# vLAR-group/DM-NeRF

Hardware: AMD Instinct MI355X
Metric: rays/sec (render) at 640x480, 64+128 samples (higher is better)
Workload: dtype f32; 1 GPU; DM-SR 'study' 640x480 synthetic camera, dm_nerf render, 64 coarse + 128 fine samples, 4096-ray chunk per step per GPU, det sampling, ins_num=13, random-init weights; chunks_per_band=75, ragged_chunk_rays=0, parallelism=ray-sharded x1

## Files before the change

dm_nerf_amd/csrc/mlp_common.h:

```cpp
#pragma once
#include <hip/hip_runtime.h>

#include <type_traits>
#include <utility>

#include "layout.h"

namespace dmn {

typedef float f32x16 __attribute__((ext_vector_type(16)));
typedef float f32x4 __attribute__((ext_vector_type(4)));

__device__ __forceinline__ f32x16 mfma32(float a, float b, f32x16 c) {
    return __builtin_amdgcn_mfma_f32_32x32x2f32(a, b, c, 0, 0, 0);
}

typedef __amdgpu_buffer_rsrc_t rsrc_t;
typedef unsigned int u32x4 __attribute__((ext_vector_type(4)));

__device__ __forceinline__ float relu1(float x) {
    const int xi = (int)__float_as_uint(x);
    return __uint_as_float((unsigned)(xi > 0 ? xi : 0));
}
__device__ __forceinline__ f32x16 relu16(f32x16 v) {
    f32x16 r;
#pragma unroll
    for (int i = 0; i < 16; ++i) r[i] = relu1(v[i]);
    return r;
}

__device__ __forceinline__ double rev_of(float v) { return (double)v * 0.15915494309189535; }

__device__ __forceinline__ double sin_rev_d(double t, int k, int quarter) {
    double g = t * (double)(1 << k) + 0.25 * (double)quarter;
    g = g - __builtin_rint(g);
    const double ag = __builtin_fabs(g);
    const double gf = ag > 0.25 ? 0.5 - ag : ag;
    const double x = gf * 6.283185307179586;
    const double x2 = x * x;
    double p = 1.0 / 1307674368000.0;
    p = __builtin_fma(p, x2, -1.0 / 6227020800.0);
    p = __builtin_fma(p, x2, 1.0 / 39916800.0);
    p = __builtin_fma(p, x2, -1.0 / 362880.0);
    p = __builtin_fma(p, x2, 1.0 / 5040.0);
    p = __builtin_fma(p, x2, -1.0 / 120.0);
    p = __builtin_fma(p, x2, 1.0 / 6.0);
    const double s = x - x * x2 * p;
    return __builtin_copysign(s, g);
}
__device__ __forceinline__ float sin_rev(double t, int k, int quarter) { return (float)sin_rev_d(t, k, quarter); }

template <int L, int NV>
__device__ __forceinline__ void encode(const float (&v)[3], f32x16 (&out)[NV], int half) {
    static_assert(NV * 16 >= 2 + 3 * L, "encoding registers too small");
#pragma unroll
    for (int i = 0; i < NV; ++i) out[i] = (f32x16)(0.f);
    out[0][0] = half ? v[1] : v[0];
    out[0][1] = half ? 0.f : v[2];
#pragma unroll
    for (int c = 0; c < 3; ++c) {
        const double t = rev_of(v[c]);
        double sn = sin_rev_d(t, 0, 0), cs = sin_rev_d(t, 0, 1);
#pragma unroll
        for (int k = 0; k < L; ++k) {
            const int p = 2 + 3 * k + c;
            out[p >> 4][p & 15] = (float)(half ? cs : sn);
            const double s_old = sn, t2 = s_old + s_old;
            sn = t2 * cs;
            cs = __builtin_fma(-t2, s_old, 1.0);
        }
    }
}

template <int L, int NV>
__device__ __forceinline__ void load_encoded(const float* __restrict__ e, f32x16 (&out)[NV], int half) {
#pragma unroll
    for (int i = 0; i < NV; ++i) out[i] = (f32x16)(0.f);
    out[0][0] = e[half];
    out[0][1] = half ? 0.f : e[2];
#pragma unroll
    for (int k = 0; k < L; ++k) {
#pragma unroll
        for (int c = 0; c < 3; ++c) {
            const int p = 2 + 3 * k + c;
            out[p >> 4][p & 15] = e[3 + 6 * k + 3 * half + c];
        }
    }
}


#ifndef DMN_STORE_AUX
#define DMN_STORE_AUX 0
#endif
#ifdef DMN_NO_ACT_STORES
#define DMN_ACT_STORE_B32(...) ((void)0)
#else
#define DMN_ACT_STORE_B32(...) __builtin_amdgcn_raw_buffer_store_b32(__VA_ARGS__)
#endif
struct RowIO {
    rsrc_t rs;
    unsigned soff;
};

__device__ __forceinline__ unsigned f2u(float x) { return __float_as_uint(x); }

__device__ __forceinline__ rsrc_t uniform_rsrc(const float* base, int64_t n_floats) {
    const unsigned long long p = reinterpret_cast<unsigned long long>(base);
    const unsigned lo = __builtin_amdgcn_readfirstlane((unsigned)p);
    const unsigned hi = __builtin_amdgcn_readfirstlane((unsigned)(p >> 32));
    const unsigned nb = __builtin_amdgcn_readfirstlane((unsigned)(n_floats * 4));
    float* q = reinterpret_cast<float*>(((unsigned long long)hi << 32) | lo);
    return __builtin_amdgcn_make_buffer_rsrc(q, 0, (int)nb, 0x00020000);
}

__device__ __forceinline__ RowIO make_rowio(const float* base, int R, int64_t Mp, int64_t blk, int lane, int ob0 = 0) {
    RowIO io;
    const unsigned long long p = reinterpret_cast<unsigned long long>(base);
    const unsigned lo = __builtin_amdgcn_readfirstlane((unsigned)p);
    const unsigned hi = __builtin_amdgcn_readfirstlane((unsigned)(p >> 32));
    float* q = reinterpret_cast<float*>(((unsigned long long)hi << 32) | lo);
    io.rs = __builtin_amdgcn_make_buffer_rsrc(q, 4, 64, 1 << 23);
    (void)Mp;
#ifdef DMN_ACT_STORE_HOT
    blk &= 7;
#endif
    io.soff = __builtin_amdgcn_readfirstlane((unsigned)(blk * R * 128 + ob0 * 4096));
    (void)lane;
    return io;
}

__device__ __forceinline__ constexpr int run_off(int b, int r) { return (32 * b + 8 * (r >> 2) + 2 * (r & 3)) * 128; }

template <int NB>
__device__ __forceinline__ void store_rows(const RowIO& io, const f32x16 (&v)[NB]) {
#pragma unroll
    for (int b = 0; b < NB; ++b) {
#pragma unroll
        for (int r = 0; r < 16; ++r)
            DMN_ACT_STORE_B32(f2u(v[b][r]), io.rs, run_off(0, r), (int)(io.soff + b * 4096), DMN_STORE_AUX);
    }
}

template <int L, int NV>
__device__ __forceinline__ void store_encoded_rows(const float* base, int64_t Mp, int64_t blk, int lane,
                                                   const f32x16 (&e)[NV]) {
    constexpr int R = 3 + 6 * L;
    const int half = lane >> 5, j = lane & 31;
    rsrc_t rs = uniform_rsrc(base, (int64_t)R * Mp);
    const int v0 = (int)((blk * R * 32 + j) * 4);
    __builtin_amdgcn_raw_buffer_store_b32(f2u(e[0][0]), rs, v0 + half * 128, 0, 0);
    if (half == 0) __builtin_amdgcn_raw_buffer_store_b32(f2u(e[0][1]), rs, v0 + 2 * 128, 0, 0);
    const int v3 = v0 + 3 * half * 128;
#pragma unroll
    for (int k = 0; k < L; ++k) {
#pragma unroll
        for (int c = 0; c < 3; ++c) {
            const int p = 2 + 3 * k + c;
            __builtin_amdgcn_raw_buffer_store_b32(f2u(e[p >> 4][p & 15]), rs, v3 + ((3 + 6 * k + c) * 128) % 4096, ((3 + 6 * k + c) * 128) / 4096 * 4096, 0);
        }
    }
}


constexpr int SLOT_FLOATS = QUARTER_FLOATS;
constexpr int RING_FLOATS = 2 * SLOT_FLOATS;
constexpr int LDS_FLOATS = RING_FLOATS + TAB_FLOATS;
constexpr int DMA_PER_QUARTER = 16;

#define DMN_GAS __attribute__((address_space(1)))
#define DMN_LAS __attribute__((address_space(3)))

struct WStream {
    rsrc_t rs;
    unsigned voff;
    float* ring;
    int wave;
    unsigned off;
    int cslot;
    f32x4 pre[8];
};

__device__ __forceinline__ void ws_init(WStream& ws, const float* blob, int64_t blob_floats, float* ring, int lane, int wave,
                                        int64_t stream_float_off) {
    ws.rs = uniform_rsrc(blob, blob_floats);
    ws.wave = __builtin_amdgcn_readfirstlane(wave);
    ws.voff = (unsigned)(lane * 16 + ws.wave * 1024);
    ws.ring = ring;
    ws.off = __builtin_amdgcn_readfirstlane((unsigned)(stream_float_off * 4));
    ws.cslot = 0;
}

__device__ __forceinline__ void ws_fetch_piece(const WStream& ws, int i) {
    float* dst = ws.ring + (ws.cslot ^ 1) * SLOT_FLOATS + ws.wave * 256 + i * 1024;
    __builtin_amdgcn_raw_ptr_buffer_load_lds(ws.rs, (DMN_LAS void*)dst, 16, (int)ws.voff, (int)(ws.off + i * 4096), 0, 0);
}
__device__ __forceinline__ void ws_fetch(WStream& ws) {
#pragma unroll
    for (int i = 0; i < DMA_PER_QUARTER; ++i) ws_fetch_piece(ws, i);
    ws.off += QUARTER_FLOATS * 4;
}

__device__ __forceinline__ void ws_fetch_first(WStream& ws) {
    ws.cslot = 1;
    ws_fetch(ws);
    ws.cslot = 0;
}

__device__ __forceinline__ unsigned lds_addr(const void* p) {
    return (unsigned)(unsigned long long)(DMN_LAS const void*)p;
}
#ifndef DMN_TILE_RC
#define DMN_TILE_RC "v"
#endif
#ifndef DMN_CARRY_RC
#define DMN_CARRY_RC DMN_TILE_RC
#endif
template <int OFF, bool CARRY = false>
__device__ __forceinline__ void lds_read16_async(f32x4& v, unsigned addr) {
    static_assert(OFF >= 0 && OFF < 65536 && OFF % 16 == 0, "ds_read_b128 offset field");
    if constexpr (CARRY) asm volatile("ds_read_b128 %0, %1 offset:%2" : "=" DMN_CARRY_RC(v) : "v"(addr), "n"(OFF));
    else asm volatile("ds_read_b128 %0, %1 offset:%2" : "=" DMN_TILE_RC(v) : "v"(addr), "n"(OFF));
}
template <class F, int... I>
__device__ __forceinline__ void static_for_impl(F&& f, std::integer_sequence<int, I...>) {
    (f(std::integral_constant<int, I>{}), ...);
}
template <int N, class F>
__device__ __forceinline__ void static_for(F&& f) {
    static_for_impl(f, std::make_integer_sequence<int, N>{});
}
template <int N, bool CARRY = false, int NV>
__device__ __forceinline__ void lds_wait(f32x4 (&v)[NV]) {
    __builtin_amdgcn_s_waitcnt(0xC07F | (N << 8));
#pragma unroll
    for (int i = 0; i < NV; ++i) {
        if constexpr (CARRY) asm volatile("" : "+" DMN_CARRY_RC(v[i]));
        else asm volatile("" : "+" DMN_TILE_RC(v[i]));
    }
}

template <int NYOUNGER = 0>
__device__ __forceinline__ void ws_handover() {
    __builtin_amdgcn_s_waitcnt(0x0F70 | (NYOUNGER & 15) | ((NYOUNGER >> 4) << 14));
    asm volatile("" ::: "memory");
    __builtin_amdgcn_s_barrier();
    asm volatile("" ::: "memory");
}

struct NoSide {
    __device__ __forceinline__ void operator()(int) const {}
};

template <int OB>
__device__ __forceinline__ void ws_prime(WStream& ws, int lane) {
    asm volatile("s_waitcnt vmcnt(0) lgkmcnt(0)" ::: "memory");
    __builtin_amdgcn_s_barrier();
    asm volatile("" ::: "memory");
    const unsigned s0 = lds_addr(ws.ring + ws.cslot * SLOT_FLOATS) + lane * 16;
    static_for<OB>([&](auto ic) {
        constexpr int ob = decltype(ic)::value;
        lds_read16_async<ob * 1024, true>(ws.pre[ob], s0);
    });
    lds_wait<0, true>(ws.pre);
}

template <int G0, int NG, int OB, int NEXT_OB, bool ZERO = false, int NSIDE = 0, int NB, class Side = NoSide>
__device__ __forceinline__ void gemm_quarter(WStream& ws, const f32x16 (&B)[NB], f32x16 (&acc)[OB], int lane, Side&& side = Side()) {
    static_assert(NB * 16 >= (G0 + NG) * 4, "B operand too small");
    static_assert(NG * OB <= 64, "more than one quarter");
    constexpr int GM = 4 * OB;
    constexpr int Q = NG * GM;
    constexpr int P = (Q / 4) / DMA_PER_QUARTER > 0 ? (Q / 4) / DMA_PER_QUARTER : 1;
    static_assert(OB + (DMA_PER_QUARTER - 1) * P < Q - GM, "DMA pieces must be issued before the last group");
    static_assert(NG >= 2 && NEXT_OB <= GM && NEXT_OB <= 8, "hand-over does not fit the last group");
    constexpr int S0 = OB + DMA_PER_QUARTER * P;
    constexpr int SP = NSIDE > 0 ? ((Q - GM - S0) / NSIDE >= 3 ? 3 : ((Q - GM - S0) / NSIDE >= 1 ? (Q - GM - S0) / NSIDE : 1)) : 1;
    static_assert(NSIDE == 0 || (S0 + (NSIDE - 1) * SP < Q - GM && NSIDE <= 63), "side operations do not fit before the last group");
    const unsigned s0 = lds_addr(ws.ring + ws.cslot * SLOT_FLOATS) + lane * 16;
    const unsigned s1 = lds_addr(ws.ring + (ws.cslot ^ 1) * SLOT_FLOATS) + lane * 16;
    f32x4 a[2][OB];
#pragma unroll
    for (int ob = 0; ob < OB; ++ob) a[0][ob] = ws.pre[ob];
    static_for<NG>([&](auto gc) {
        constexpr int gl = decltype(gc)::value;
        lds_wait<0>(a[gl & 1]);
        if constexpr (gl == NG - 1 && NEXT_OB > 0) ws_handover<NSIDE>();
        __builtin_amdgcn_sched_barrier(0);
        static_for<GM>([&](auto ic) {
            constexpr int i = decltype(ic)::value;
            constexpr int kk = i / OB, ob = i % OB, M = gl * GM + i;
            constexpr int p = (G0 + gl) * 4 + kk;
            if constexpr (gl + 1 < NG && i < OB)
                lds_read16_async<((gl + 1) * OB + i) * 1024>(a[(gl + 1) & 1][i], s0);
            if constexpr (gl == NG - 1 && i < NEXT_OB) lds_read16_async<i * 1024, true>(ws.pre[i], s1);
            if constexpr (M >= OB && (M - OB) % P == 0 && (M - OB) / P < DMA_PER_QUARTER) ws_fetch_piece(ws, (M - OB) / P);
            if constexpr (NSIDE > 0 && M >= S0 && (M - S0) % SP == 0 && (M - S0) / SP < NSIDE) side((M - S0) / SP);
            if constexpr (ZERO && G0 + gl == 0 && kk == 0) acc[ob] = mfma32(a[gl & 1][ob][kk], B[p >> 4][p & 15], (f32x16)(0.f));
            else acc[ob] = mfma32(a[gl & 1][ob][kk], B[p >> 4][p & 15], acc[ob]);
            __builtin_amdgcn_sched_barrier(0);
        });
    });
    if constexpr (NEXT_OB > 0) __builtin_amdgcn_s_waitcnt(0xC07F);
    ws.off += QUARTER_FLOATS * 4;
    ws.cslot ^= 1;
}

template <int OB>
__device__ __forceinline__ void init_bias_lds(const float* tab_seg, f32x16 (&acc)[OB], int half) {
#pragma unroll
    for (int ob = 0; ob < OB; ++ob) {
        const f32x4* b4 = reinterpret_cast<const f32x4*>(tab_seg + (ob * 2 + half) * 16);
#pragma unroll
        for (int q = 0; q < 4; ++q) {
            const f32x4 v = b4[q];
            acc[ob][4 * q + 0] = v[0]; acc[ob][4 * q + 1] = v[1];
            acc[ob][4 * q + 2] = v[2]; acc[ob][4 * q + 3] = v[3];
        }
    }
}

template <int NB>
__device__ __forceinline__ void pack_mask(const f32x16 (&h)[NB], unsigned (&m)[NB / 2]) {
#pragma unroll
    for (int w = 0; w < NB / 2; ++w) m[w] = 0;
#pragma unroll
    for (int i = 0; i < 32; ++i) {
#pragma unroll
        for (int w = 0; w < NB / 2; ++w) {
            const int p = 32 * w + i;
            const float x = h[p >> 4][p & 15];
            asm volatile("v_cmp_lt_f32 vcc, 0, %1\n\tv_addc_co_u32 %0, vcc, %0, %0, vcc" : "+v"(m[w]) : "v"(x) : "vcc");
        }
    }
}

template <int NB>
__device__ __forceinline__ void apply_mask(f32x16 (&d)[NB], const unsigned (&m)[NB / 2], const f32x16 (&g)[NB]) {
#pragma unroll
    for (int p = 0; p < NB * 16; ++p) {
        const unsigned keep = (unsigned)__builtin_amdgcn_sbfe((int)m[p >> 5], 31 - (p & 31), 1);
        d[p >> 4][p & 15] = __uint_as_float(__float_as_uint(g[p >> 4][p & 15]) & keep);
    }
}

template <int NB>
__device__ __forceinline__ void store_row_one(const RowIO& io, const f32x16 (&v)[NB], int p) {
    DMN_ACT_STORE_B32(f2u(v[p >> 4][p & 15]), io.rs, run_off(0, p & 15), (int)(io.soff + (p >> 4) * 4096), DMN_STORE_AUX);
}

template <int P0, int NP, int NB>
__device__ __forceinline__ void store_rows_part(const RowIO& io, const f32x16 (&v)[NB]) {
#pragma unroll
    for (int p = P0; p < P0 + NP; ++p)
        DMN_ACT_STORE_B32(f2u(v[p >> 4][p & 15]), io.rs, run_off(0, p & 15), (int)(io.soff + (p >> 4) * 4096), DMN_STORE_AUX);
}

}
```

dm_nerf_amd/csrc/mlp_fwd_density.hip:

```cpp
#include <hip/hip_runtime.h>

#include "../../include/dmnerf_hip.h"
#include "common.h"
#include "layout.h"
#include "mlp_common.h"

using namespace dmn;

namespace {

constexpr int DENSITY_QUARTERS = 1 + 5 * 4 + 1 + 2 * 4 + 1;
static_assert(DENSITY_QUARTERS <= N_QUARTERS - 2 * 4, "the look-ahead quarter must exist in the fused-heads blob as well");

struct DensityArgs {
    const float* blob;
    BlobLayout L;
    const float* rays_o;
    const float* rays_d;
    const float* z;
    float* sigma;
    int64_t M;
    int S;
};

__global__ __launch_bounds__(256) void mlp_fwd_density_kernel(const DensityArgs a) {
    extern __shared__ __attribute__((aligned(16))) float lds[];
    float* const tab = lds + RING_FLOATS;
    const int lane = threadIdx.x & 63;
    const int half = lane >> 5;
    const int wave = __builtin_amdgcn_readfirstlane(threadIdx.x >> 6);
    const int64_t nblk = (a.M + 31) / 32;
    const int64_t blk_raw = (int64_t)blockIdx.x * 4 + wave;
    const int64_t blk = blk_raw < nblk ? blk_raw : nblk - 1;
    auto fresh = [](int x) -> int { asm volatile("" : "+v"(x)); return x; };
    const int64_t m_in = blk * 32 + (lane & 31);
    const int64_t m = m_in < a.M ? m_in : a.M - 1;

    const float* __restrict__ blob = a.blob;
    const BlobLayout& L = a.L;

    float pt[3];
    {
        const int64_t n = m / a.S;
        const float ox = a.rays_o[n * 3 + 0], oy = a.rays_o[n * 3 + 1], oz = a.rays_o[n * 3 + 2];
        const float dx = a.rays_d[n * 3 + 0], dy = a.rays_d[n * 3 + 1], dz = a.rays_d[n * 3 + 2];
        const float zv = a.z[m];
        pt[0] = ox + dx * zv; pt[1] = oy + dy * zv; pt[2] = oz + dz * zv;
    }
    f32x16 pe[2];
    f32x4 tabv[TAB_FLOATS / 1024];
    {
        const f32x4* src = reinterpret_cast<const f32x4*>(blob) + threadIdx.x;
#pragma unroll
        for (int k = 0; k < TAB_FLOATS / 1024; ++k) tabv[k] = src[k * 256];
    }
    WStream ws;
    ws_init(ws, blob, L.stream + (int64_t)DENSITY_QUARTERS * QUARTER_FLOATS, lds, lane, wave, L.stream);
    ws_fetch_first(ws);
    encode<POS_L, 2>(pt, pe, half);
    {
        f32x4* dst = reinterpret_cast<f32x4*>(tab) + threadIdx.x;
#pragma unroll
        for (int k = 0; k < TAB_FLOATS / 1024; ++k) dst[k * 256] = tabv[k];
    }

    f32x16 h[8], acc[8];
    ws_prime<8>(ws, lane);
    init_bias_lds<8>(tab + L.b0, acc, half);
    gemm_quarter<0, 8, 8, 8>(ws, pe, acc, lane);
#pragma unroll
    for (int b = 0; b < 8; ++b) h[b] = relu16(acc[b]);

#pragma nounroll
    for (int st = 0; st < 7; ++st) {
        init_bias_lds<8>(tab + L.b_stage + st * (int)bias_floats(8), acc, half);
        gemm_quarter<0, 8, 8, 8>(ws, h, acc, lane);
        gemm_quarter<8, 8, 8, 8>(ws, h, acc, lane);
        gemm_quarter<16, 8, 8, 8>(ws, h, acc, lane);
        gemm_quarter<24, 8, 8, 8>(ws, h, acc, lane);
        if (st == 4) {
            gemm_quarter<0, 8, 8, 8>(ws, pe, acc, lane);
        }
#pragma unroll
        for (int b = 0; b < 8; ++b) h[b] = relu16(acc[b]);
    }
    const f32x4* wd = reinterpret_cast<const f32x4*>(tab + L.w_den + fresh(half) * 128);
    float part = 0.f;
#pragma unroll
    for (int i = 0; i < 32; ++i) {
        const f32x4 w = wd[i];
#pragma unroll
        for (int j = 0; j < 4; ++j) {
            const int p = 4 * i + j;
            part = fmaf(h[p >> 4][p & 15], w[j], part);
        }
    }
    const float sigma = part + __shfl_xor(part, 32) + tab[L.b_den];
    const int64_t ms = blk * 32 + (fresh(lane) & 31);
    if (ms < a.M && fresh(half) == 0) a.sigma[ms] = sigma;
}

}

extern "C" int dmnerf_mlp_fwd_rays_density(const float* d_blob, int ins_num, const float* d_rays_o,
                                           const float* d_rays_d, const float* d_z, int64_t N, int S,
                                           float* d_sigma, void* stream) {
    if (ins_num < 1 || ins_num + 1 > DMNERF_MAX_LOGITS) return dmn_fail(DMNERF_E_ARG, "mlp_fwd_rays_density: ins_num %d unsupported", ins_num);
    if (N < 0 || S < 1) return dmn_fail(DMNERF_E_ARG, "mlp_fwd_rays_density: bad N=%lld S=%d", (long long)N, S);
    if (N == 0) return DMNERF_OK;
    if (!d_blob || !d_rays_o || !d_rays_d || !d_z || !d_sigma) return dmn_fail(DMNERF_E_ARG, "mlp_fwd_rays_density: null pointer");
    DensityArgs a{};
    a.blob = d_blob; a.L = make_layout(ins_num); a.rays_o = d_rays_o; a.rays_d = d_rays_d; a.z = d_z;
    a.sigma = d_sigma; a.M = N * S; a.S = S;
    const int64_t nblk = (a.M + 31) / 32;
    const int64_t grid = (nblk + 3) / 4;
    if (grid > 0x7fffffffLL) return dmn_fail(DMNERF_E_ARG, "mlp_fwd_rays_density: %lld samples is too many for one launch", (long long)a.M);
    constexpr size_t lds_bytes = (size_t)LDS_FLOATS * sizeof(float);
    static DmnOncePerDevice once;
    if (hipError_t e = once.run([] { return hipFuncSetAttribute((const void*)mlp_fwd_density_kernel,
                                                                hipFuncAttributeMaxDynamicSharedMemorySize, (int)lds_bytes); }); e != hipSuccess)
        return dmn_fail_hip(e, "mlp_fwd_rays_density: hipFuncSetAttribute");
    hipLaunchKernelGGL(mlp_fwd_density_kernel, dim3((unsigned)grid), dim3(256), lds_bytes, (hipStream_t)stream, a);
    return dmn_check_launch("mlp_fwd_rays_density");
}
```

dm_nerf_amd/csrc/mlp_fwd_impl.h:

```cpp
#pragma once
#include <hip/hip_runtime.h>

#include "../../include/dmnerf_hip.h"
#include "common.h"
#include "layout.h"
#include "mlp_common.h"

#ifdef DMN_FWD_TRACE
extern long long* g_dmn_fwd_trace;
#endif

using namespace dmn;

namespace {

constexpr int PARK_FLOATS = 4096;

struct MlpArgs {
    const float* blob;
    BlobLayout L;
    const float* rays_o;
    const float* rays_d;
    const float* z;
    const float* x;
    float* raw;
    float* save;
    int64_t M;
    int S;
#ifdef DMN_FWD_TRACE
    long long* trace;
#endif
};
#ifdef DMN_FWD_TRACE
#define DMN_STAMP(k) do { if (a.trace && threadIdx.x == 0) { a.trace[8 * blockIdx.x + (k)] = (long long)clock64(); if ((k) == 0) a.trace[8 * blockIdx.x + 7] = (long long)wall_clock64(); } } while (0)
#else
#define DMN_STAMP(k) do {} while (0)
#endif

template <int OBI, bool EMBEDDED, bool SAVE, bool FUSED = false>
__global__ __launch_bounds__(256) void mlp_fwd_kernel(const MlpArgs a) {
    extern __shared__ __attribute__((aligned(16))) float lds[];
    float* const tab = lds + RING_FLOATS;
    DMN_STAMP(0);
    const int lane = threadIdx.x & 63;
    const int half = lane >> 5;
    const int wave = __builtin_amdgcn_readfirstlane(threadIdx.x >> 6);
    const int64_t nblk = (a.M + 31) / 32;
    const int64_t blk_raw = (int64_t)blockIdx.x * 4 + wave;
    const bool wave_active = blk_raw < nblk;
    const int64_t blk = wave_active ? blk_raw : nblk - 1;
    auto fresh = [](int x) -> int { asm volatile("" : "+v"(x)); return x; };
    auto sample_of_lane = [&]() -> int64_t { return blk * 32 + (fresh(lane) & 31); };
    const int64_t m_in = blk * 32 + (lane & 31);
    const int64_t m = m_in < a.M ? m_in : a.M - 1;
    auto park = [&]() -> f32x4* { return reinterpret_cast<f32x4*>(lds + LDS_FLOATS + wave * (PARK_FLOATS / 4)) + lane; };

    const float* __restrict__ blob = a.blob;
    const BlobLayout& L = a.L;

    float pt[3], vd[3];
    const float* xr = nullptr;
    if constexpr (EMBEDDED) {
        xr = a.x + m * (POS_CH + DIR_CH);
    } else {
        const int64_t n = m / a.S;
        const float ox = a.rays_o[n * 3 + 0], oy = a.rays_o[n * 3 + 1], oz = a.rays_o[n * 3 + 2];
        const float dx = a.rays_d[n * 3 + 0], dy = a.rays_d[n * 3 + 1], dz = a.rays_d[n * 3 + 2];
        const float zv = a.z[m];
        pt[0] = ox + dx * zv; pt[1] = oy + dy * zv; pt[2] = oz + dz * zv;
        const float nrm = sqrtf(dx * dx + dy * dy + dz * dz);
        vd[0] = dx / nrm; vd[1] = dy / nrm; vd[2] = dz / nrm;
    }
    f32x16 pe[2];
    f32x16 de[1];
    if constexpr (EMBEDDED) {
        load_encoded<POS_L, 2>(xr, pe, half);
        load_encoded<DIR_L, 1>(xr + POS_CH, de, half);
    }
    f32x4 tabv[TAB_FLOATS / 1024];
    {
        const f32x4* src = reinterpret_cast<const f32x4*>(blob) + threadIdx.x;
#pragma unroll
        for (int k = 0; k < TAB_FLOATS / 1024; ++k) tabv[k] = src[k * 256];
    }
    WStream ws;
    ws_init(ws, blob, L.total, lds, lane, wave, L.stream);
    ws_fetch_first(ws);
    if constexpr (!EMBEDDED) {
        encode<POS_L, 2>(pt, pe, half);
        encode<DIR_L, 1>(vd, de, half);
    }
    {
        f32x4* dst = reinterpret_cast<f32x4*>(tab) + threadIdx.x;
#pragma unroll
        for (int k = 0; k < TAB_FLOATS / 1024; ++k) dst[k * 256] = tabv[k];
    }

    const SaveLayout SL = make_save_layout(a.M);
    const int64_t MP = save_row_len(a.M);
    const int srows = 1;
    rsrc_t bits_rs;
    int bits_voff = 0;
    if constexpr (SAVE) {
        bits_rs = uniform_rsrc(a.save + SL.bits, (int64_t)srows * (BITS_WORDS_PER_BLOCK / 32) * MP);
        bits_voff = (int)((blk * BITS_WORDS_PER_BLOCK + lane * 4) * 4);
    }

    DMN_STAMP(1);
    f32x16 h[8], acc[8];
    auto save_mask8 = [&](int layer) {
        unsigned m[4];
        pack_mask<8>(h, m);
        u32x4 v = {m[0], m[1], m[2], m[3]};
        __builtin_amdgcn_raw_buffer_store_b128(v, bits_rs, bits_voff + layer * 1024, 0, 0);
    };
    ws_prime<8>(ws, lane);
    if constexpr (SAVE) {
        store_encoded_rows<POS_L, 2>(a.save + SL.pe, srows * MP, blk, lane, pe);
        store_encoded_rows<DIR_L, 1>(a.save + SL.de, srows * MP, blk, lane, de);
    }
#pragma unroll
    for (int q = 0; q < 4; ++q) {
        const f32x4 v = {de[0][4 * q + 0], de[0][4 * q + 1], de[0][4 * q + 2], de[0][4 * q + 3]};
        park()[q * 64] = v;
    }
    init_bias_lds<8>(tab + L.b0, acc, half);
    gemm_quarter<0, 8, 8, 8>(ws, pe, acc, lane);
#pragma unroll
    for (int b = 0; b < 8; ++b) h[b] = relu16(acc[b]);
    if constexpr (SAVE) save_mask8(0);

    DMN_STAMP(2);
    float sigma = 0.f, rgb_out[3] = {0.f, 0.f, 0.f};

    auto stage = [&](int st, auto next_ob, auto save_h) {
        constexpr int NEXT = decltype(next_ob)::value;
        constexpr bool SAVE_H = SAVE && decltype(save_h)::value;
        RowIO hio;
        if constexpr (SAVE) hio = make_rowio(a.save + SL.h + (int64_t)(st < 8 ? st : 7) * 256 * MP, 256, (st < 8 ? srows : 0) * MP, blk, lane);
        init_bias_lds<8>(tab + L.b_stage + st * (int)bias_floats(8), acc, half);
        constexpr int NS = SAVE_H ? 43 : 0;
        auto st_h = [&](int k0) { return [&, k0](int k) { store_row_one(hio, h, k0 + k); }; };
        gemm_quarter<0, 8, 8, 8>(ws, h, acc, lane);
        gemm_quarter<8, 8, 8, 8, false, NS>(ws, h, acc, lane, st_h(0));
        gemm_quarter<16, 8, 8, 8, false, NS>(ws, h, acc, lane, st_h(43));
        gemm_quarter<24, 8, 8, NEXT, false, SAVE_H ? 42 : 0>(ws, h, acc, lane, st_h(86));
    };
    typedef std::integral_constant<int, 8> Next8;
    typedef std::integral_constant<int, 4> Next4;

#pragma nounroll
    for (int st = 0; st < 7; ++st) {
        stage(st, Next8{}, std::true_type{});
        if (st == 4) {
            gemm_quarter<0, 8, 8, 8>(ws, pe, acc, lane);
        }
#pragma unroll
        for (int b = 0; b < 8; ++b) h[b] = relu16(acc[b]);
        if constexpr (SAVE) save_mask8(st + 1);
    }
    {
        const f32x4* wd = reinterpret_cast<const f32x4*>(tab + L.w_den + fresh(half) * 128);
        float part = 0.f;
#pragma unroll
        for (int i = 0; i < 32; ++i) {
            const f32x4 w = wd[i];
#pragma unroll
            for (int j = 0; j < 4; ++j) {
                const int p = 4 * i + j;
                part = fmaf(h[p >> 4][p & 15], w[j], part);
            }
        }
        sigma = part + __shfl_xor(part, 32) + tab[L.b_den];
        asm volatile("" : "+v"(sigma));
    }

    DMN_STAMP(3);
    if constexpr (!FUSED) stage(7, Next4{}, std::true_type{});
    {
        f32x16 hid[4];
        init_bias_lds<4>(tab + L.b_rgbh, hid, half);
        auto& fsrc = *(FUSED ? &h : &acc);
        constexpr bool SAVE_H7 = SAVE && FUSED;
        RowIO h7io;
        if constexpr (SAVE_H7) h7io = make_rowio(a.save + SL.h + (int64_t)7 * 256 * MP, 256, srows * MP, blk, lane);
        auto st_h7 = [&](int k0) { return [&, k0](int k) { store_row_one(h7io, h, k0 + k); }; };
        gemm_quarter<0, 16, 4, 4, false, SAVE_H7 ? 63 : 0>(ws, fsrc, hid, lane, st_h7(0));
        gemm_quarter<16, 16, 4, 4, false, SAVE_H7 ? 63 : 0>(ws, fsrc, hid, lane, st_h7(63));
        f32x16 dpk[1];
#pragma unroll
        for (int q = 0; q < 4; ++q) {
            const f32x4 v = park()[q * 64];
            dpk[0][4 * q + 0] = v[0]; dpk[0][4 * q + 1] = v[1]; dpk[0][4 * q + 2] = v[2]; dpk[0][4 * q + 3] = v[3];
        }
        gemm_quarter<0, 4, 4, 8, false, SAVE_H7 ? 2 : 0>(ws, dpk, hid, lane, st_h7(126));
#pragma unroll
        for (int b = 0; b < 4; ++b) hid[b] = relu16(hid[b]);
        if constexpr (SAVE) {
            store_rows<4>(make_rowio(a.save + SL.g1, 128, srows * MP, blk, lane), hid);
            unsigned m[2];
            pack_mask<4>(hid, m);
            __builtin_amdgcn_raw_buffer_store_b32(m[0], bits_rs, (int)((blk * BITS_WORDS_PER_BLOCK + 2048 + lane * 2) * 4), 0, 0);
            __builtin_amdgcn_raw_buffer_store_b32(m[1], bits_rs, (int)((blk * BITS_WORDS_PER_BLOCK + 2048 + lane * 2 + 1) * 4), 0, 0);
        }
#pragma unroll
        for (int c = 0; c < 3; ++c) {
            const f32x4* wr = reinterpret_cast<const f32x4*>(tab + L.w_rgbo + (c * 2 + fresh(half)) * 64);
            float part = 0.f;
#pragma unroll
            for (int i = 0; i < 16; ++i) {
                const f32x4 w = wr[i];
#pragma unroll
                for (int j = 0; j < 4; ++j) {
                    const int p = 4 * i + j;
                    part = fmaf(hid[p >> 4][p & 15], w[j], part);
                }
            }
            rgb_out[c] = part + __shfl_xor(part, 32) + tab[L.b_rgbo + c];
            asm volatile("" : "+v"(rgb_out[c]));
        }
    }

    if constexpr (!FUSED) stage(8, Next4{}, std::false_type{});
    {
        f32x16 hid[4];
        init_bias_lds<4>(tab + L.b_insh, hid, half);
        auto& qsrc = *(FUSED ? &h : &acc);
        gemm_quarter<0, 16, 4, 4>(ws, qsrc, hid, lane);
        gemm_quarter<16, 16, 4, OBI>(ws, qsrc, hid, lane);
#pragma unroll
        for (int b = 0; b < 4; ++b) hid[b] = relu16(hid[b]);
        constexpr int NS3 = SAVE ? (OBI == 1 ? 43 : 63) : 0;
        RowIO g2io;
        if constexpr (SAVE) {
            g2io = make_rowio(a.save + SL.g2, 128, srows * MP, blk, lane);
            store_rows_part<NS3, 64 - NS3>(g2io, hid);
            unsigned m[2];
            pack_mask<4>(hid, m);
            __builtin_amdgcn_raw_buffer_store_b32(m[0], bits_rs, (int)((blk * BITS_WORDS_PER_BLOCK + 2176 + lane * 2) * 4), 0, 0);
            __builtin_amdgcn_raw_buffer_store_b32(m[1], bits_rs, (int)((blk * BITS_WORDS_PER_BLOCK + 2176 + lane * 2 + 1) * 4), 0, 0);
        }
        f32x16 io[OBI];
        init_bias_lds<OBI>(tab + L.b_inso, io, half);
        auto st_3 = [&](int k) { store_row_one(g2io, hid, k); };
        gemm_quarter<0, 16, OBI, 0, false, NS3>(ws, hid, io, lane, st_3);
        const int64_t ms = sample_of_lane();
        const int hf = fresh(half);
        float* __restrict__ out_row = a.raw + (ms < a.M ? ms : a.M - 1) * (4 + L.C);
        if (ms < a.M) {
#pragma unroll
            for (int b = 0; b < OBI; ++b) {
#pragma unroll
                for (int r = 0; r < 16; ++r) {
                    const int ch = 32 * b + (r & 3) + 8 * (r >> 2) + 4 * hf;
                    if (ch < L.C) out_row[4 + ch] = io[b][r];
                }
            }
        }
    }
    DMN_STAMP(4);
    const int64_t ms = sample_of_lane();
    float* __restrict__ out_row = a.raw + (ms < a.M ? ms : a.M - 1) * (4 + L.C);
    if (ms < a.M && fresh(half) == 0) {
        out_row[0] = rgb_out[0];
        out_row[1] = rgb_out[1];
        out_row[2] = rgb_out[2];
        out_row[3] = sigma;
    }
    DMN_STAMP(5);
}

template <bool EMBEDDED, bool SAVE, bool FUSED = false>
int launch(const MlpArgs& a, hipStream_t stream) {
    const int64_t nblk = (a.M + 31) / 32;
    const int64_t grid = (nblk + 3) / 4;
    if (grid > 0x7fffffffLL) return dmn_fail(DMNERF_E_ARG, "mlp_fwd: %lld samples is too many for one launch", (long long)a.M);
    if (SAVE && a.M > DMNERF_MAX_TRAIN_SAMPLES)
        return dmn_fail(DMNERF_E_ARG, "mlp_fwd_train: %lld samples per launch exceed %lld (32-bit row offsets); split the batch",
                        (long long)a.M, (long long)DMNERF_MAX_TRAIN_SAMPLES);
    dim3 g((unsigned)grid), b(256);
    constexpr size_t lds_bytes = (size_t)(LDS_FLOATS + PARK_FLOATS) * sizeof(float);
#define DMN_LAUNCH(OBI_)                                                                                              \
    {                                                                                                                \
        static DmnOncePerDevice once;                                                                                 \
        if (hipError_t e_ = once.run([] { return hipFuncSetAttribute((const void*)(mlp_fwd_kernel<OBI_, EMBEDDED, SAVE, FUSED>),              \
                                                     hipFuncAttributeMaxDynamicSharedMemorySize, (int)lds_bytes); }); e_ != hipSuccess) \
            return dmn_fail_hip(e_, "mlp_fwd: hipFuncSetAttribute");                                       \
        hipLaunchKernelGGL((mlp_fwd_kernel<OBI_, EMBEDDED, SAVE, FUSED>), g, b, lds_bytes, stream, a);                       \
    }
    switch (a.L.OBI) {
        case 1: DMN_LAUNCH(1) break;
        case 2: DMN_LAUNCH(2) break;
        case 3: DMN_LAUNCH(3) break;
        case 4: DMN_LAUNCH(4) break;
        default: return dmn_fail(DMNERF_E_ARG, "mlp_fwd: unsupported logit count C=%d", a.L.C);
    }
#undef DMN_LAUNCH
    return dmn_check_launch("mlp_fwd");
}

}
```

Baseline: 445,700 rays/s.

## Fuse ReLU and next-layer bias init into the last MFMA group of each layer

Adds a LayerTail hook to gemm_quarter. In the final k-group it reorders MFMAs to output-block-major and interleaves the ReLU and the next stage's bias load into the gaps between MFMAs, using a skew so each block finishes before it is read. The hidden-layer loop is restructured so the last quarter of every stage (or the skip-connection quarter at stage 4) carries this tail, and the separate relu16 and init_bias_lds passes go away. This aims to hide the per-layer epilogue VALU/LDS latency behind matrix work, at the cost of more complex scheduling and tighter register and skew constraints. It applies only to the non-save, non-fused, non-embedded forward path and to the density kernel.

Result: slower. 439,600 rays/s (-1.4%).

```diff
diff --git a/dm_nerf_amd/csrc/mlp_common.h b/dm_nerf_amd/csrc/mlp_common.h
--- a/dm_nerf_amd/csrc/mlp_common.h
+++ b/dm_nerf_amd/csrc/mlp_common.h
@@ -251,6 +251,33 @@
     __device__ __forceinline__ void operator()(int) const {}
 };
 
+struct NoTail {
+    static constexpr int ITEMS = 0, SKEW = 0;
+    template <int T>
+    __device__ __forceinline__ void operator()(std::integral_constant<int, T>) const {}
+};
+template <int OB, bool BIAS>
+struct LayerTail {
+    static constexpr int ITEMS = 4 * OB;
+    static constexpr int SKEW = BIAS ? 7 : 5;
+    f32x16 (&acc)[OB];
+    f32x16 (&h)[OB];
+    const f32x4* bias;
+    __device__ __forceinline__ LayerTail(f32x16 (&acc_)[OB], f32x16 (&h_)[OB], const float* tab_seg = nullptr, int half = 0)
+        : acc(acc_), h(h_), bias(reinterpret_cast<const f32x4*>(tab_seg + half * 16)) {}
+    template <int T>
+    __device__ __forceinline__ void operator()(std::integral_constant<int, T>) {
+        constexpr int ob = T / 4, q = T % 4;
+#pragma unroll
+        for (int j = 0; j < 4; ++j) h[ob][4 * q + j] = relu1(acc[ob][4 * q + j]);
+        if constexpr (BIAS) {
+            const f32x4 v = bias[ob * 8 + q];
+            acc[ob][4 * q + 0] = v[0]; acc[ob][4 * q + 1] = v[1];
+            acc[ob][4 * q + 2] = v[2]; acc[ob][4 * q + 3] = v[3];
+        }
+    }
+};
+
 template <int OB>
 __device__ __forceinline__ void ws_prime(WStream& ws, int lane) {
     asm volatile("s_waitcnt vmcnt(0) lgkmcnt(0)" ::: "memory");
@@ -264,8 +291,11 @@
     lds_wait<0, true>(ws.pre);
 }
 
-template <int G0, int NG, int OB, int NEXT_OB, bool ZERO = false, int NSIDE = 0, int NB, class Side = NoSide>
-__device__ __forceinline__ void gemm_quarter(WStream& ws, const f32x16 (&B)[NB], f32x16 (&acc)[OB], int lane, Side&& side = Side()) {
+template <int G0, int NG, int OB, int NEXT_OB, bool ZERO = false, int NSIDE = 0, int NB, class Side = NoSide, class Tail = NoTail>
+__device__ __forceinline__ void gemm_quarter(WStream& ws, const f32x16 (&B)[NB], f32x16 (&acc)[OB], int lane, Side&& side = Side(),
+                                             Tail&& tail = Tail()) {
+    typedef std::remove_reference_t<Tail> TailT;
+    constexpr bool TAIL = !std::is_same_v<TailT, NoTail>;
     static_assert(NB * 16 >= (G0 + NG) * 4, "B operand too small");
     static_assert(NG * OB <= 64, "more than one quarter");
     constexpr int GM = 4 * OB;
@@ -288,19 +318,29 @@
         __builtin_amdgcn_sched_barrier(0);
         static_for<GM>([&](auto ic) {
             constexpr int i = decltype(ic)::value;
-            constexpr int kk = i / OB, ob = i % OB, M = gl * GM + i;
+            constexpr bool OBMAJOR = TAIL && gl == NG - 1;
+            constexpr int kk = OBMAJOR ? i % 4 : i / OB, ob = OBMAJOR ? i / 4 : i % OB, M = gl * GM + i;
             constexpr int p = (G0 + gl) * 4 + kk;
             if constexpr (gl + 1 < NG && i < OB)
                 lds_read16_async<((gl + 1) * OB + i) * 1024>(a[(gl + 1) & 1][i], s0);
             if constexpr (gl == NG - 1 && i < NEXT_OB) lds_read16_async<i * 1024, true>(ws.pre[i], s1);
             if constexpr (M >= OB && (M - OB) % P == 0 && (M - OB) / P < DMA_PER_QUARTER) ws_fetch_piece(ws, (M - OB) / P);
             if constexpr (NSIDE > 0 && M >= S0 && (M - S0) % SP == 0 && (M - S0) / SP < NSIDE) side((M - S0) / SP);
+            if constexpr (OBMAJOR) {
+                if constexpr (i >= TailT::SKEW) tail(std::integral_constant<int, i - TailT::SKEW>{});
+            }
             if constexpr (ZERO && G0 + gl == 0 && kk == 0) acc[ob] = mfma32(a[gl & 1][ob][kk], B[p >> 4][p & 15], (f32x16)(0.f));
             else acc[ob] = mfma32(a[gl & 1][ob][kk], B[p >> 4][p & 15], acc[ob]);
             __builtin_amdgcn_sched_barrier(0);
         });
     });
     if constexpr (NEXT_OB > 0) __builtin_amdgcn_s_waitcnt(0xC07F);
+    if constexpr (TAIL) {
+        static_assert(NSIDE == 0 && TailT::SKEW < GM && TailT::ITEMS >= GM - TailT::SKEW, "layer tail does not fit the last group");
+        static_for<TailT::ITEMS - (GM - TailT::SKEW)>([&](auto tc) {
+            tail(std::integral_constant<int, GM - TailT::SKEW + decltype(tc)::value>{});
+        });
+    }
     ws.off += QUARTER_FLOATS * 4;
     ws.cslot ^= 1;
 }
diff --git a/dm_nerf_amd/csrc/mlp_fwd_density.hip b/dm_nerf_amd/csrc/mlp_fwd_density.hip
--- a/dm_nerf_amd/csrc/mlp_fwd_density.hip
+++ b/dm_nerf_amd/csrc/mlp_fwd_density.hip
@@ -67,22 +67,23 @@
     f32x16 h[8], acc[8];
     ws_prime<8>(ws, lane);
     init_bias_lds<8>(tab + L.b0, acc, half);
-    gemm_quarter<0, 8, 8, 8>(ws, pe, acc, lane);
-#pragma unroll
-    for (int b = 0; b < 8; ++b) h[b] = relu16(acc[b]);
+    auto stage_bias = [&](int st) -> const float* { return tab + L.b_stage + st * (int)bias_floats(8); };
+    auto tail8 = [&](int next_st) { return LayerTail<8, true>(acc, h, stage_bias(next_st), fresh(half)); };
+    gemm_quarter<0, 8, 8, 8>(ws, pe, acc, lane, NoSide(), tail8(0));
 
 #pragma nounroll
     for (int st = 0; st < 7; ++st) {
-        init_bias_lds<8>(tab + L.b_stage + st * (int)bias_floats(8), acc, half);
         gemm_quarter<0, 8, 8, 8>(ws, h, acc, lane);
         gemm_quarter<8, 8, 8, 8>(ws, h, acc, lane);
         gemm_quarter<16, 8, 8, 8>(ws, h, acc, lane);
-        gemm_quarter<24, 8, 8, 8>(ws, h, acc, lane);
+        f32x16 bq[2];
         if (st == 4) {
-            gemm_quarter<0, 8, 8, 8>(ws, pe, acc, lane);
+            gemm_quarter<24, 8, 8, 8>(ws, h, acc, lane);
+            bq[0] = pe[0]; bq[1] = pe[1];
+        } else {
+            bq[0] = h[6]; bq[1] = h[7];
         }
-#pragma unroll
-        for (int b = 0; b < 8; ++b) h[b] = relu16(acc[b]);
+        gemm_quarter<0, 8, 8, 8>(ws, bq, acc, lane, NoSide(), tail8(st + 1));
     }
     const f32x4* wd = reinterpret_cast<const f32x4*>(tab + L.w_den + fresh(half) * 128);
     float part = 0.f;
diff --git a/dm_nerf_amd/csrc/mlp_fwd_impl.h b/dm_nerf_amd/csrc/mlp_fwd_impl.h
--- a/dm_nerf_amd/csrc/mlp_fwd_impl.h
+++ b/dm_nerf_amd/csrc/mlp_fwd_impl.h
@@ -125,9 +125,16 @@
         park()[q * 64] = v;
     }
     init_bias_lds<8>(tab + L.b0, acc, half);
-    gemm_quarter<0, 8, 8, 8>(ws, pe, acc, lane);
-#pragma unroll
-    for (int b = 0; b < 8; ++b) h[b] = relu16(acc[b]);
+    constexpr bool TAILED = !EMBEDDED && !SAVE && !FUSED;
+    auto stage_bias = [&](int st) -> const float* { return tab + L.b_stage + st * (int)bias_floats(8); };
+    [[maybe_unused]] auto tail8 = [&](int next_st) { return LayerTail<8, true>(acc, h, stage_bias(next_st), fresh(half)); };
+    if constexpr (TAILED) {
+        gemm_quarter<0, 8, 8, 8>(ws, pe, acc, lane, NoSide(), tail8(0));
+    } else {
+        gemm_quarter<0, 8, 8, 8>(ws, pe, acc, lane);
+#pragma unroll
+        for (int b = 0; b < 8; ++b) h[b] = relu16(acc[b]);
+    }
     if constexpr (SAVE) save_mask8(0);
 
     DMN_STAMP(2);
@@ -138,7 +145,7 @@
         constexpr bool SAVE_H = SAVE && decltype(save_h)::value;
         RowIO hio;
         if constexpr (SAVE) hio = make_rowio(a.save + SL.h + (int64_t)(st < 8 ? st : 7) * 256 * MP, 256, (st < 8 ? srows : 0) * MP, blk, lane);
-        init_bias_lds<8>(tab + L.b_stage + st * (int)bias_floats(8), acc, half);
+        if (!(TAILED && st == 7)) init_bias_lds<8>(stage_bias(st), acc, half);
         constexpr int NS = SAVE_H ? 43 : 0;
         auto st_h = [&](int k0) { return [&, k0](int k) { store_row_one(hio, h, k0 + k); }; };
         gemm_quarter<0, 8, 8, 8>(ws, h, acc, lane);
@@ -149,15 +156,32 @@
     typedef std::integral_constant<int, 8> Next8;
     typedef std::integral_constant<int, 4> Next4;
 
+    if constexpr (TAILED) {
 #pragma nounroll
-    for (int st = 0; st < 7; ++st) {
-        stage(st, Next8{}, std::true_type{});
-        if (st == 4) {
-            gemm_quarter<0, 8, 8, 8>(ws, pe, acc, lane);
-        }
-#pragma unroll
-        for (int b = 0; b < 8; ++b) h[b] = relu16(acc[b]);
-        if constexpr (SAVE) save_mask8(st + 1);
+        for (int st = 0; st < 7; ++st) {
+            gemm_quarter<0, 8, 8, 8>(ws, h, acc, lane);
+            gemm_quarter<8, 8, 8, 8>(ws, h, acc, lane);
+            gemm_quarter<16, 8, 8, 8>(ws, h, acc, lane);
+            f32x16 bq[2];
+            if (st == 4) {
+                gemm_quarter<24, 8, 8, 8>(ws, h, acc, lane);
+                bq[0] = pe[0]; bq[1] = pe[1];
+            } else {
+                bq[0] = h[6]; bq[1] = h[7];
+            }
+            gemm_quarter<0, 8, 8, 8>(ws, bq, acc, lane, NoSide(), tail8(st + 1));
+        }
+    } else {
+#pragma nounroll
+        for (int st = 0; st < 7; ++st) {
+            stage(st, Next8{}, std::true_type{});
+            if (st == 4) {
+                gemm_quarter<0, 8, 8, 8>(ws, pe, acc, lane);
+            }
+#pragma unroll
+            for (int b = 0; b < 8; ++b) h[b] = relu16(acc[b]);
+            if constexpr (SAVE) save_mask8(st + 1);
+        }
     }
     {
         const f32x4* wd = reinterpret_cast<const f32x4*>(tab + L.w_den + fresh(half) * 128);
@@ -193,9 +217,13 @@
             const f32x4 v = park()[q * 64];
             dpk[0][4 * q + 0] = v[0]; dpk[0][4 * q + 1] = v[1]; dpk[0][4 * q + 2] = v[2]; dpk[0][4 * q + 3] = v[3];
         }
-        gemm_quarter<0, 4, 4, 8, false, SAVE_H7 ? 2 : 0>(ws, dpk, hid, lane, st_h7(126));
-#pragma unroll
-        for (int b = 0; b < 4; ++b) hid[b] = relu16(hid[b]);
+        if constexpr (TAILED) {
+            gemm_quarter<0, 4, 4, 8>(ws, dpk, hid, lane, NoSide(), LayerTail<4, false>(hid, hid));
+        } else {
+            gemm_quarter<0, 4, 4, 8, false, SAVE_H7 ? 2 : 0>(ws, dpk, hid, lane, st_h7(126));
+#pragma unroll
+            for (int b = 0; b < 4; ++b) hid[b] = relu16(hid[b]);
+        }
         if constexpr (SAVE) {
             store_rows<4>(make_rowio(a.save + SL.g1, 128, srows * MP, blk, lane), hid);
             unsigned m[2];
@@ -227,9 +255,13 @@
         init_bias_lds<4>(tab + L.b_insh, hid, half);
         auto& qsrc = *(FUSED ? &h : &acc);
         gemm_quarter<0, 16, 4, 4>(ws, qsrc, hid, lane);
-        gemm_quarter<16, 16, 4, OBI>(ws, qsrc, hid, lane);
-#pragma unroll
-        for (int b = 0; b < 4; ++b) hid[b] = relu16(hid[b]);
+        if constexpr (TAILED) {
+            gemm_quarter<16, 16, 4, OBI>(ws, qsrc, hid, lane, NoSide(), LayerTail<4, false>(hid, hid));
+        } else {
+            gemm_quarter<16, 16, 4, OBI>(ws, qsrc, hid, lane);
+#pragma unroll
+            for (int b = 0; b < 4; ++b) hid[b] = relu16(hid[b]);
+        }
         constexpr int NS3 = SAVE ? (OBI == 1 ? 43 : 63) : 0;
         RowIO g2io;
         if constexpr (SAVE) {
```
